# ScissorJack-ever/AlayaLite

Measured on AMD Instinct MI355X. Metric: QPS @ recall@10>=0.95, GIST-960 L2, 1M base / 1k queries, higher is better.
Workload: dtype f32

## Files before the change

alayalite_amd/csrc/capi.cpp:

```cpp
#include "../../include/alaya_hip.h"

#include <hip/hip_runtime_api.h>

#include <algorithm>
#include <cfloat>
#include <cmath>
#include <cstring>
#include <memory>
#include <mutex>
#include <stdexcept>
#include <limits>
#include <string>
#include <thread>
#include <vector>

#include "build_kernels.h"
#include "graph_update.h"
#include "hnsw_build.h"
#include "flat_bound.h"
#include "flat_kernels.h"
#include <cstdlib>
#include "screen_bound.h"
#include "search_kernels.h"

// ... 100 lines not shown
  uint32_t hash_log2_override = 0;
  int helpers_mode = -1;
  DevBuf help_stats;
  uint64_t help_stats_slots = 0;
  struct ScreenCopy {
    DevBuf rows, err;
    uint64_t cap = 0;
    bool ready = false;
    bool failed = false;
  };
  ScreenCopy screen_copy[2];
  uint32_t screen_format = 0;
  DevBuf screen_stats;
  uint64_t screen_stats_slots = 0;
  uint32_t last_grid = 0, last_waves = 0;
  int visited_mode_override = 0;
  int num_cus = 0;
  uint64_t capacity = 0;
  std::unique_ptr<alaya_amd::HostGraph> upd_graph;
  std::unique_ptr<alaya_amd::RowMirror> upd_rows;
  std::unique_ptr<alaya_amd::UpdateContext> upd_ctx;
  hipStream_t stream = nullptr;
  hipEvent_t scratch_ev = nullptr;
  hipStream_t scratch_stream = nullptr;
  bool scratch_used = false;
  uint64_t device_bytes() const {
    return base.bytes + valid.bytes + l0.bytes + levels.bytes + upper_off.bytes +
           upper_edges.bytes + eps.bytes + overflow.bytes + dirty.bytes + stab.bytes + codes.bytes + sq_min.bytes +
           sq_max.bytes;
  }
// ... 229 lines not shown
      const size_t probe = search_wave_lds_bytes(ix->stride, ef, 12, true);
      hip_check(search_occupancy(resolve_search_variant(r), p.ip, 1, probe, &b1), "occupancy");
      const uint64_t resident1 = static_cast<uint64_t>(std::max(1, b1)) * static_cast<uint64_t>(stream_cus(ix, stream));
      if (nq > resident1 && 2 * nq <= 3 * resident1) r.want |= kModeTwoWaves;
    }
  }
  if (ensure_screen(ix, p, p.sq8_order == 0 && plain, stream)) r.want |= kModeScreen;
  return r;
}

struct SearchPlan {
  const alaya_amd::SearchVariant *variant;
  int W;
  size_t lds;
  int grid;
};

SearchPlan plan_search(alaya_index *ix, SearchParams &p, alaya_amd::SearchRequest r, uint64_t nq, uint32_t ef,
                       hipStream_t stream) {
  using namespace alaya_amd;
  SearchPlan plan{};
  for (;;) {
    plan.variant = &resolve_search_variant(r);
    const int mode = plan.variant->mode;
    if ((r.want & kModeStamp) != 0 && (mode & kModeStamp) == 0)
      throw ArgError("no stamped search kernel for dim " + std::to_string(ix->dim) +
                     (p.sq8_order ? " SQ8 (order " + std::to_string(p.sq8_order) + ")" : std::string(" f32")) +
                     ": see the variant list in search_variants.h");
    p.help = (mode & kModeHelp) != 0;
    p.two_waves = (mode & kModeTwoWaves) != 0;
    p.screen = (mode & kModeScreen) != 0 ? ix->screen_format : 0u;
// ... 14 lines not shown
        fits = false;
      }
    }
    plan.lds = search_shared_lds_bytes(ix->stride, p.sq8_order != 0) + static_cast<size_t>(plan.W) * p.wave_lds +
               (p.help ? kHelpBoardBytes : 0);
    if (!p.help || (fits && plan.lds <= kLdsPerCu)) break;
    r.want &= ~kModeHelp;
  }
  if (plan.lds > kLdsPerCu) throw ArgError("ef / dim too large for the LDS budget");
  int per_cu = 0;
  hip_check(search_occupancy(*plan.variant, p.ip, plan.W, plan.lds, &per_cu), "occupancy");
  per_cu = static_cast<int>(std::max<uint64_t>(1, std::min<uint64_t>(per_cu, max_search_waves_per_cu() / plan.W)));
  const uint64_t cus = static_cast<uint64_t>(stream_cus(ix, stream));
  const uint64_t blocks_needed = p.help ? static_cast<uint64_t>(per_cu) * cus : (nq + plan.W - 1) / plan.W;
  plan.grid = static_cast<int>(std::max<uint64_t>(1, std::min<uint64_t>(blocks_needed, static_cast<uint64_t>(per_cu) * cus)));
  return plan;
}

void do_search(alaya_index *ix, const float *d_q, uint64_t nq, uint32_t k, uint32_t ef,
               uint32_t *d_ids, float *d_dists, uint32_t *d_cnt, hipStream_t stream,
               uint64_t *d_stamps = nullptr, bool sq8 = false, uint32_t fill_id = 0) {
  if (!ix->base.ptr) throw ArgError("index has no base vectors");
  if (!ix->has_graph) throw ArgError("index has no graph");
  if (ef == 0) throw ArgError("ef must be >= 1");
  if (k == 0 || nq == 0) return;
  if (ix->graph_n > ix->n) throw ArgError("graph has more nodes than base vectors");
  SearchParams p = base_params(ix);
  p.l0 = ix->l0.as<uint32_t>();
  p.R = ix->R;
  p.dedup_edges = ix->dedup;
// ... 23 lines not shown
    p.sq_max = ix->sq_max.as<float>();
  }
  p.stab_log2 = spill_table_log2(p.sq8_order, std::max<uint32_t>(1, ceil_log2(std::max<uint64_t>(ix->n, 2))), ef);
  if (const char *e = std::getenv("ALAYA_HELP_FLAGS")) p.help_flags = static_cast<uint32_t>(std::strtoul(e, nullptr, 10));
  const SearchPlan plan = plan_search(ix, p, search_request(ix, p, nq, ef, stream), nq, ef, stream);
  if (p.screen >= 2) {
    p.screen_u8 = ix->screen_copy[1].rows.as<uint8_t>();
  } else if (p.screen) {
    p.screen_rows = ix->screen_copy[0].rows.as<uint16_t>();
    p.screen_err = ix->screen_copy[0].err.as<float>();
  }
  scratch_acquire(ix, stream);
  const uint64_t searchers = static_cast<uint64_t>(plan.grid) * plan.W;
  prepare_spill(ix, p, searchers, stream);
  ix->last_grid = static_cast<uint32_t>(plan.grid);
  ix->last_waves = static_cast<uint32_t>(plan.W);
  ix->help_stats_slots = p.help ? searchers : 0;
  if (p.help) {
    ix->help_stats.reserve(searchers * 12);
    p.help_stats = ix->help_stats.as<uint32_t>();
  }
  ix->screen_stats_slots = p.screen ? searchers : 0;
  if (p.screen) {
    ix->screen_stats.reserve(searchers * 8);
    p.screen_stats = ix->screen_stats.as<uint32_t>();
  }
  ix->work.reserve(4);
  p.work_counter = ix->work.as<uint32_t>();
  hip_check(hipMemsetAsync(p.work_counter, 0, 4, stream), "hipMemsetAsync");
  hip_check(alaya_amd::launch_search(*plan.variant, p, plan.grid, plan.W, plan.lds, stream), "search launch");
  scratch_release(ix, stream);
}

uint32_t screen_default(uint32_t dim) {
  return (dim == 512 || dim == 768 || dim == 960 || dim == 1024) ? 3u : 0u;
}

void screen_fill(alaya_index *ix, uint32_t format, uint64_t first, uint64_t count, hipStream_t stream) {
  alaya_index::ScreenCopy &c = ix->screen_copy[format - 1];
  hip_check(format == 2 ? alaya_amd::launch_screen_rows_u8(ix->base.as<float>(), first, count, ix->stride,
                                                           c.rows.as<uint8_t>(), stream)
                        : alaya_amd::launch_screen_rows(ix->base.as<float>(), first, count, ix->stride,
                                                        c.rows.as<uint16_t>(), c.err.as<float>(), stream),
            "screening copy");
}
// ... 1449 lines not shown

int alaya_stream_destroy(void *stream) {
  return guarded([&] {
    if (stream) hip_check(hipStreamDestroy(static_cast<hipStream_t>(stream)), "hipStreamDestroy");
  });
}

int alaya_index_last_launch(const alaya_index *ix, uint32_t *workgroups, uint32_t *waves_per_group) {
  return guarded([&] {
    if (!ix) throw ArgError("null index");
    if (workgroups) *workgroups = ix->last_grid;
    if (waves_per_group) *waves_per_group = ix->last_waves;
  });
}

int alaya_index_set_helpers(alaya_index *ix, int mode) {
  return guarded([&] {
    if (!ix) throw ArgError("null index");
    if (mode < -1 || mode > 1) throw ArgError("helpers mode must be -1 (automatic), 0 (off) or 1 (on)");
    ix->helpers_mode = mode;
  });
}

int alaya_index_help_stats(alaya_index *ix, uint64_t *memo_dists, uint64_t *memo_expansions, uint64_t *helper_rows) {
  return guarded_scratch(ix, [&] {
    if (!ix) throw ArgError("null index");
    uint64_t m = 0, x = 0, r = 0;
    if (ix->help_stats_slots) {
      set_device(ix);
      scratch_drain(ix);
// ... 174 lines not shown
```

alayalite_amd/csrc/pybind_module.cpp:

```cpp
#include <pybind11/numpy.h>
#include <pybind11/pybind11.h>
#include <pybind11/stl.h>

#include <algorithm>
#include <cmath>
#include <cstring>
#include <fstream>
#include <memory>
#include <queue>
#include <stdexcept>
#include <string>
#include <vector>

#include "../../include/alaya_hip.h"

extern "C" int alaya_index_flat_diag(alaya_index *, const float *, uint64_t, uint32_t, int, uint32_t *, float *,
                                     uint32_t *, uint32_t *, void *);
#include "host_distance.h"

namespace py = pybind11;

namespace alaya_py {

enum class IndexType { FLAT = 0, HNSW = 1, NSG = 2, FUSION = 3, QG = 4 };
// ... 253 lines not shown
  void set_helpers(int m) { check(alaya_index_set_helpers(ix_, m)); }
  py::tuple last_launch() {
    uint32_t g = 0, w = 0;
    check(alaya_index_last_launch(ix_, &g, &w));
    return py::make_tuple(g, w);
  }
  py::tuple help_stats() {
    uint64_t m = 0, x = 0, r = 0;
    check(alaya_index_help_stats(ix_, &m, &x, &r));
    return py::make_tuple(m, x, r);
  }
  py::tuple screen_stats() {
    uint64_t a = 0, b = 0;
    check(alaya_index_screen_stats(ix_, &a, &b));
    return py::make_tuple(a, b);
  }
  void set_rerank_mode(int m) {
    if (m != 1 && m != 2) throw std::invalid_argument("rerank mode must be 1 (reference) or 2 (corrected)");
    rerank_mode_ = m;
  }
  int rerank_mode() const { return rerank_mode_; }
  py::array device_distances(py::array queries, py::array_t<uint32_t> ids) {
    py::array q = prepare_queries(queries);
    py::array_t<uint32_t, py::array::c_style | py::array::forcecast> idc(ids);
    const uint64_t nq = q.shape(0);
    const uint32_t n = static_cast<uint32_t>(idc.size());
    py::array_t<float> out({static_cast<py::ssize_t>(nq), static_cast<py::ssize_t>(n)});
    check(alaya_index_distances(ix_, static_cast<const float *>(q.data()), nq, idc.data(), n,
                                out.mutable_data()));
    return out;
// ... 544 lines not shown
  py::tuple last_launch() {
    uint32_t g = 0, w = 0;
    check(alaya_index_last_launch(ix_, &g, &w));
    return py::make_tuple(g, w);
  }
  py::tuple help_stats() {
    uint64_t m = 0, x = 0, r = 0;
    check(alaya_index_help_stats(ix_, &m, &x, &r));
    return py::make_tuple(m, x, r);
  }
  py::tuple screen_stats() {
    uint64_t a = 0, b = 0;
    check(alaya_index_screen_stats(ix_, &a, &b));
    return py::make_tuple(a, b);
  }
  py::tuple profile_search(py::array_t<float, py::array::c_style | py::array::forcecast> q, uint32_t k,
                           uint32_t ef, int space) {
    const uint64_t nq = q.shape(0);
    py::array_t<uint32_t> ids({static_cast<py::ssize_t>(nq), static_cast<py::ssize_t>(k)});
    py::array_t<uint32_t> c({static_cast<py::ssize_t>(nq), static_cast<py::ssize_t>(4)});
    py::array_t<uint64_t> st({static_cast<py::ssize_t>(nq), static_cast<py::ssize_t>(8)});
    check(alaya_index_profile_search(ix_, q.data(), nq, k, ef, space, ids.mutable_data(), c.mutable_data(),
                                     st.mutable_data()));
    return py::make_tuple(ids, c, st);
  }
  uint64_t device_bytes() const {
    uint64_t b = 0;
    check(alaya_index_info(ix_, nullptr, nullptr, nullptr, nullptr, &b));
    return b;
  }
// ... 65 lines not shown
      .def("batch_search_with_distance", &PyIndexInterface::batch_search_with_distance,
           py::arg("queries"), py::arg("topk"), py::arg("ef"), py::arg("num_threads"))
      .def("exact_search", &PyIndexInterface::exact_search, py::arg("queries"), py::arg("topk"))
      .def("save", &PyIndexInterface::save, py::arg("index_path"), py::arg("data_path"),
           py::arg("quant_path") = std::string())
      .def("load", &PyIndexInterface::load, py::arg("index_path"), py::arg("data_path"),
           py::arg("quant_path") = std::string())
      .def("get_data_dim", &PyIndexInterface::get_data_dim)
      .def("last_counters", &PyIndexInterface::last_counters)
      .def("set_hash_log2", &PyIndexInterface::set_hash_log2)
      .def("set_visited_mode", &PyIndexInterface::set_visited_mode)
      .def("set_helpers", &PyIndexInterface::set_helpers)
      .def("last_launch", &PyIndexInterface::last_launch)
      .def("help_stats", &PyIndexInterface::help_stats)
      .def("screen_stats", &PyIndexInterface::screen_stats)
      .def("set_rerank_mode", &PyIndexInterface::set_rerank_mode)
      .def("rerank_mode", &PyIndexInterface::rerank_mode)
      .def("device_distances", &PyIndexInterface::device_distances)
      .def("graph_arrays", &PyIndexInterface::graph_arrays);


  py::class_<Graph, std::shared_ptr<Graph>>(m, "Graph")
      .def_static("build", &Graph::build, py::arg("data"), py::arg("metric") = 0, py::arg("R") = 32u,
                  py::arg("ef_construction") = 100u, py::arg("num_threads") = 1u, py::arg("seed") = 100u)
      .def_static("load", &Graph::load, py::arg("path"), py::arg("id_bytes") = 4)
      .def_static("from_arrays", &Graph::from_arrays, py::arg("l0"), py::arg("levels"), py::arg("upper_off"),
                  py::arg("upper_edges"), py::arg("upper_R"), py::arg("ep"), py::arg("eps") = py::none())
      .def("save", &Graph::save, py::arg("path"), py::arg("id_bytes") = 4, py::arg("capacity") = 0u)
      .def("arrays", &Graph::arrays);
  py::class_<DeviceIndex, std::shared_ptr<DeviceIndex>>(m, "DeviceIndex")
      .def(py::init<int>(), py::arg("device") = 0)
      .def("set_base", &DeviceIndex::set_base, py::arg("rows"), py::arg("metric") = 0, py::arg("valid") = py::none())
      .def("set_graph", &DeviceIndex::set_graph)
      .def("build_graph", &DeviceIndex::build_graph, py::arg("R") = 32, py::arg("ef_construction") = 100,
           py::arg("seed") = 100, py::arg("batch_div") = 0, py::arg("max_batch") = 0, py::arg("refine") = 2)
      .def("search", &DeviceIndex::search, py::arg("queries"), py::arg("k"), py::arg("ef"))
      .def("search_device", &DeviceIndex::search_device)
      .def("shard_search_device", &DeviceIndex::shard_search_device)
      .def("distances", &DeviceIndex::distances)
      .def("set_hash_log2", &DeviceIndex::set_hash_log2)
      .def("set_visited_mode", &DeviceIndex::set_visited_mode)
      .def("set_helpers", &DeviceIndex::set_helpers)
      .def("last_launch", &DeviceIndex::last_launch)
      .def("help_stats", &DeviceIndex::help_stats)
      .def("screen_stats", &DeviceIndex::screen_stats)
      .def("flat_search", &DeviceIndex::flat_search, py::arg("queries"), py::arg("k"))
      .def("flat_search_device", &DeviceIndex::flat_search_device)
      .def("flat_diag", &DeviceIndex::flat_diag)
      .def("flat_contraction", &DeviceIndex::flat_contraction)
      .def("search_sq8_device", &DeviceIndex::search_sq8_device)
      .def("shard_search_sq8_device", &DeviceIndex::shard_search_sq8_device)
      .def("set_sq8", &DeviceIndex::set_sq8, py::arg("codes"), py::arg("min"), py::arg("max"), py::arg("order") = 2)
      .def("search_sq8", &DeviceIndex::search_sq8, py::arg("queries"), py::arg("k"), py::arg("ef"),
           py::arg("rerank") = 1, py::arg("rerank_queries") = py::none())
      .def("profile_search", &DeviceIndex::profile_search, py::arg("q"), py::arg("k"), py::arg("ef"),
           py::arg("space") = 0)
      .def("device_bytes", &DeviceIndex::device_bytes);
  m.def("sq8_train", [](py::array_t<float, py::array::c_style | py::array::forcecast> data) {
    const uint32_t d = static_cast<uint32_t>(data.shape(1));
    py::array_t<float> mn(d), mx(d);
// ... 103 lines not shown
```

alayalite_amd/csrc/search_device.h:

```cpp
#pragma once
#include <hip/hip_runtime.h>

#include <cfloat>
#include <cstdint>

#include "screen_bound.h"
#include "search_kernels.h"

namespace alaya_amd {
namespace {

constexpr uint32_t kEmpty = 0xffffffffu;
constexpr uint32_t kChecked = 0x80000000u;
constexpr uint32_t kIdMask = 0x7fffffffu;

__device__ __forceinline__ int lane_id() { return __lane_id(); }

__device__ __forceinline__ void wave_sync() {
  __builtin_amdgcn_fence(__ATOMIC_SEQ_CST, "wavefront");
  __builtin_amdgcn_wave_barrier();
}

__device__ __forceinline__ uint64_t ballot(bool p) { return __ballot(p); }

// ... 479 lines not shown
  Q.a2 = read_lane(a2, 0) + read_lane(a2, 32);
  Q.lo = lo;
  Q.scale = scale;
  Q.err = screen_u8_err(read_lane(sum, 0) + read_lane(sum, 32), p.stride, bad);
  return Q;
}

template <int kXor, int kN>
__device__ __forceinline__ void screen_fold(uint32_t *v, bool upper) {
#pragma unroll
  for (int i = 0; i < kN / 2; ++i) {
    const uint32_t keep = upper ? v[i + kN / 2] : v[i];
    const uint32_t send = upper ? v[i] : v[i + kN / 2];
    v[i] = keep + lane_xor<kXor>(send);
  }
}

template <int kChunks, typename Hook>
__device__ __forceinline__ void screen_dots_int(const SearchParams &p, const uint4 qc, const uint32_t *ids, int n,
                                                uint32_t *out, Hook after_issue) {
  constexpr int kPieces = 2 * kChunks;
  const int lane = lane_id();
  const uint32_t rec = screen_u8_record_bytes(p.stride);
  const uint32_t piece = kScreenU8Header + 16u * static_cast<uint32_t>(lane < kPieces ? lane : kPieces - 1);
  const int mine = ((lane & 1) << 4) | ((lane & 2) << 2) | (lane & 4) | ((lane & 8) >> 2) | ((lane & 16) >> 4);
  for (int base = 0; base < n; base += 32) {
    const uint32_t id = ids[base + lane < n ? base + lane : base];
    uint4 y[32];
#pragma unroll
    for (int r = 0; r < 32; ++r) {
// ... 807 lines not shown
```

alayalite_amd/csrc/search_kernels.h:

```cpp
#pragma once
#include <hip/hip_runtime_api.h>

#include <cstddef>
#include <cstdint>

#include "search_variants.h"

namespace alaya_amd {

struct SearchParams {
  const float *base;
  uint64_t n;
  uint32_t dim;
  uint32_t stride;
  const uint32_t *valid;
  bool ip;
  bool generic;
  const uint32_t *l0;
  uint32_t R;
  bool dedup_edges;
  const uint32_t *levels;
  const uint64_t *upper_off;
  const uint32_t *upper_edges;
  uint32_t upper_R;
// ... 27 lines not shown
  int sq8_order;
  const uint8_t *codes;
  uint32_t code_stride;
  const float *sq_min;
  const float *sq_max;
  uint32_t help;
  uint32_t help_flags;
  uint32_t memo_off;
  uint32_t two_waves;
  uint32_t *help_stats;
  uint32_t screen;
  const uint16_t *screen_rows;
  const float *screen_err;
  const uint8_t *screen_u8;
  uint32_t *screen_stats;
};

struct RerankParams {
  const uint32_t *search_ids;
  uint32_t k;
  uint32_t n_src;
  uint32_t n_take;
  uint32_t zeros;
  uint32_t fill_id;
  uint32_t *out_ids;
  float *out_dists;
};

constexpr uint32_t kVisWide = 0xffffffffu;
constexpr size_t kHelpBoardBytes = 256;
#ifndef ALAYA_HELP_DEPTH
// ... 29 lines not shown
```

alayalite_amd/csrc/search_kernels.hip:

```cpp
#include <hip/hip_runtime.h>

#include <cfloat>
#include <cstdint>

#include "screen_bound.h"
#include "search_kernels.h"
#include "search_device.h"

#ifndef ALAYA_MIN_WAVES_SQ8
#define ALAYA_MIN_WAVES_SQ8 -1
#endif
#ifndef ALAYA_MIN_WAVES_NARROW
#define ALAYA_MIN_WAVES_NARROW 0
#endif
#ifndef ALAYA_MIN_WAVES_WIDE
#define ALAYA_MIN_WAVES_WIDE 0
#endif
template <int kSpace>
constexpr bool space_sq8() { return kSpace == 1 || kSpace == 2; }
template <int kSpace>
constexpr bool space_tab() { return kSpace == 2; }

template <int kChunks, int kSpace, int kMode = 0>
constexpr int search_min_waves() {
// ... 425 lines not shown
      if (want) L.cid[slot] = v;
      wave_sync();
      space_distances<kIP, kChunks, kSpace>(p, Lt, L.cid, n, L.cd);
      if (lane == 0) b->own[wave].rows += static_cast<uint32_t>(n);
      if (want) {
        const uint64_t e = (static_cast<uint64_t>(seq) << 32) | __float_as_uint(L.cd[slot]);
        __hip_atomic_store(memo + (static_cast<uint32_t>(t) * kHelpSlots + s) * R + lane, e, __ATOMIC_RELAXED,
                           __HIP_MEMORY_SCOPE_WORKGROUP);
      }
      wave_sync();
    }
    if (!worked) __builtin_amdgcn_s_sleep(4);
  }
}

template <bool kIP, int kChunks, int kMode, int kSpace = 0>
__global__ void __launch_bounds__(256)
    __attribute__((amdgpu_waves_per_eu(search_min_waves<kChunks, kSpace, kMode>() ? search_min_waves<kChunks, kSpace, kMode>() : 1,
                                       8))) hnsw_search_kernel(SearchParams p) {
  extern __shared__ __attribute__((aligned(16))) unsigned char smem[];
  constexpr bool kStamp = (kMode & kModeStamp) != 0;
  constexpr bool kCheck = (kMode & kModeCheck) != 0;
  constexpr bool kHelp = (kMode & kModeHelp) != 0;
  constexpr int kRows = (kMode & kModeTwoWaves) != 0 ? 1 : 0;
  constexpr bool kScreen = (kMode & kModeScreen) != 0;
  static_assert(!kScreen || (kSpace == 0 && !kIP && !kHelp && kChunks >= 16 && kChunks % 2 == 0), "screen: wide f32 L2 rows");
  constexpr int kScreenRows = (kMode & kModeTwoWaves) != 0 ? 2 : 4;
  constexpr int kScreenRowsU8 = 4;
  uint32_t n_screened = 0, n_screened_out = 0;
  const int lane = lane_id();
  const int wave = static_cast<int>(threadIdx.x >> 6);
  const int W = static_cast<int>(blockDim.x >> 6);
  const Lds L = carve_lds<kSpace>(p, smem, wave);
  fill_shared<kSpace>(p, L);
  HelpBoard *board = kHelp ? help_board(p, smem, W) : nullptr;
  HelpMine mine;
  if constexpr (kHelp) {
    if constexpr (ALAYA_HELP_PRIO > 0) __builtin_amdgcn_s_setprio(ALAYA_HELP_PRIO);
    if (threadIdx.x == 0) help_board_init(board);
    __syncthreads();
    for (int s = 0; s < kHelpSlots; ++s) mine.node[s] = kEmpty, mine.seq[s] = 0u;
    mine.next_seq = 0u;
    mine.memo_wave = -1;
  }
  const uint64_t bit_words = (p.n + 31) / 32;
  const uint64_t slot = static_cast<uint64_t>(blockIdx.x) * (blockDim.x >> 6) + wave;
  uint32_t *slot_bits = p.overflow_bits + slot * bit_words;
  uint32_t *slot_dirty = p.dirty_words + slot * p.dirty_cap;
  uint16_t *slot_stab = (space_tab<kSpace>() && p.spill_table) ? p.spill_table + (slot << p.stab_log2) : nullptr;

  bool first_round = true;
  for (;;) {
    uint32_t qi = 0;
    if (kHelp && first_round) {
      qi = static_cast<uint32_t>(wave) * gridDim.x + blockIdx.x;
    } else {
      if (lane == 0) qi = atomicAdd(p.work_counter, 1u);
      qi = read_lane(qi, 0) + (kHelp ? static_cast<uint32_t>(W) * gridDim.x : 0u);
    }
    first_round = false;
    if (qi >= p.nq) break;
    if constexpr (kHelp) mine_reset(board, wave, mine);

    uint64_t st[8] = {0, 0, 0, 0, 0, 0, 0, 0};
    uint64_t t_prev = kStamp ? __builtin_readcyclecounter() : 0;
    const uint64_t t_begin = t_prev;
    auto stamp = [&](int slot) {
      if constexpr (kStamp) {
        const uint64_t now = __builtin_readcyclecounter();
        st[slot] += now - t_prev;
        t_prev = now;
      }
    };
    Visited vs;
    PoolState ps;
    uint32_t n_dist = 0, n_expand = 0, n_dist_up = 0, n_hops_up = 0;
    query_begin<kIP, kChunks, kSpace, kRows>(p, L, qi, slot_bits, slot_dirty, slot_stab, vs, ps, n_dist_up, n_hops_up);
    ScreenQuery sq{};
    if constexpr (kScreen) {
      if (p.screen == 3) sq = screen_query_codes<kChunks>(p, L.q);
    }

    stamp(0);
    uint32_t pred = kEmpty, pred_v = kEmpty;
    constexpr bool kSpillPrefetch = kSpace != 0;
    constexpr bool kRegMerge = kSpace == 0 && kChunks > 0 && kChunks <= 8;
    uint32_t pre_u = kEmpty;
    uint64_t pre_lo = 0ull, pre_hi = 0ull;
    while (ps.cur < ps.size) {
      uint32_t c1 = kEmpty, c2 = kEmpty;
      const uint32_t u = pool_pop<kHelp>(ps, L, &c1, &c2);
      ++n_expand;
      uint32_t look = 0u;
      if constexpr (kHelp) {
        if (mine.memo_wave < 0 && (n_expand & 3u) == 1u) {
          const uint32_t hw = help_word(board);
          if ((hw >> 8) != 0u) mine.memo_wave = static_cast<int>(hw >> 8) - 1;
        }
        if (mine.memo_wave >= 0) {
#pragma unroll
          for (int hs = 0; hs < kHelpSlots; ++hs)
            if (mine.node[hs] == u) look = (mine.seq[hs] << 2) | static_cast<uint32_t>(hs);
          mine_request(board, wave, mine, u, c1, c2);
        }
      }
#ifndef ALAYA_FINE_STAMPS
      if (kStamp && vs.spilled) st[5]++;
// ... 38 lines not shown
      }
      pre_u = kEmpty;
      pre_lo = pre_hi = 0ull;
      const uint64_t fm = ballot(fresh);
      const int nf = __popcll(fm);
      pred = ps.cur < ps.size ? (L.pi[ps.cur] & kIdMask) : kEmpty;
      if (pred != kEmpty && lane < static_cast<int>(p.R)) pred_v = p.l0[static_cast<uint64_t>(pred) * p.R + lane];
#ifdef ALAYA_FINE_STAMPS
      stamp(5);
#else
      stamp(2);
#endif
      if (nf == 0) continue;
      const uint32_t slot = __popcll(fm & ((1ull << lane) - 1ull));
      if (fresh) L.cid[slot] = v;
      const uint32_t *dist_ids = L.cid;
      bool compute = true;
      if constexpr (kHelp) {
        if (look != 0u) {
          const uint32_t seq = look >> 2;
          const int hs = static_cast<int>(look & 3u);
          const uint64_t *memo = help_memo<kSpace>(p, smem, mine.memo_wave) +
                                 (static_cast<uint32_t>(wave) * kHelpSlots + hs) * p.R;
          uint64_t e = 0ull;
          if (fresh) e = __hip_atomic_load(memo + lane, __ATOMIC_RELAXED, __HIP_MEMORY_SCOPE_WORKGROUP);
          const bool got = fresh && static_cast<uint32_t>(e >> 32) == seq;
          help_retire(board, wave, hs, seq);
          uint32_t *ids2 = reinterpret_cast<uint32_t *>(L.sd);
          if (fresh) {
            ids2[slot] = got ? kEmpty : v;
// ... 14 lines not shown
          if (vs.spilled && pred != kEmpty && !(p.spill_flags & 1u)) {
            if (p.spill_flags & 4u) __builtin_amdgcn_s_waitcnt(0);
            spill_prefetch(vs, pred_v, lane < static_cast<int>(p.R), pre_lo, pre_hi);
            pre_u = pred;
          }
        }
      };
      int nd = nf;
      if constexpr (kScreen) {
        if (ps.size == ps.ef) {
          const float tau = L.pd[ps.size - 1];
          const bool in = lane < nf;
          const uint32_t c = in ? L.cid[lane] : 0u;
          float e_row = 0.f;
          float lb3 = 0.f;
          if (p.screen == 3) {
            const uint8_t *rp = p.screen_u8 + static_cast<uint64_t>(c) * screen_u8_record_bytes(p.stride);
            const float4 head = *reinterpret_cast<const float4 *>(rp);
            const uint2 sums = *reinterpret_cast<const uint2 *>(rp + screen_u8_sums_offset(p.stride));
            screen_dots_int<kChunks>(p, sq.codes, L.cid, nf, reinterpret_cast<uint32_t *>(L.cd), second_level_prefetch);
            lb3 = screen_int_bound(p.stride, sq.err, sq.lo, sq.scale, sq.a1, sq.a2, head.x, head.y, head.z, sums.x, sums.y,
                                   __float_as_uint(L.cd[lane]));
          } else if (p.screen == 2) {
            if (in) e_row = *reinterpret_cast<const float *>(p.screen_u8 + static_cast<uint64_t>(c) * screen_u8_record_bytes(p.stride));
            screen_distances_u8<kChunks, kScreenRowsU8>(p, L.q, L.cid, nf, L.cd, second_level_prefetch);
          } else {
            if (in) e_row = p.screen_err[c];
            screen_distances<kChunks, kScreenRows>(p, L.q, L.cid, nf, L.cd, second_level_prefetch);
          }
          bool keep = false;
          if (in) {
// ... 30 lines not shown
      stamp(3);
      n_dist += nf;
      const bool has = lane < nd;
      const uint32_t cid = has ? L.cid[lane] : 0u;
      const float cd = has ? L.cd[lane] : 0.f;
      wave_sync();
      pool_merge<kRegMerge>(ps, L, has, cid, cd, [&](uint32_t nx) {
        if (nx != pred) {
          const uint32_t old_pred = pred;
          (void)old_pred;
          pred = nx;
          if (lane < static_cast<int>(p.R)) pred_v = p.l0[static_cast<uint64_t>(nx) * p.R + lane];
          if constexpr (kHelp) {
            if (mine.memo_wave >= 0) mine_request(board, wave, mine, kEmpty, nx, old_pred);
          }
        }
      }
#ifdef ALAYA_FINE_STAMPS
      , [&]() { stamp(7); }
#endif
      );
      stamp(4);
    }

    query_end(p, L, ps, qi, n_dist, n_expand, n_dist_up, n_hops_up);
    visit_end(vs);
    if constexpr (kStamp) {
      st[6] = __builtin_readcyclecounter() - t_begin;
      if (lane < 8) p.stamps[static_cast<uint64_t>(qi) * 8 + lane] = st[lane & 7];
    }
    wave_sync();
  }
  if constexpr (kHelp) {
    help_siblings<kIP, kChunks, kSpace>(p, smem, L, board, wave, W);
    if (p.help_stats != nullptr && lane == 0) {
      p.help_stats[3 * slot] = board->own[wave].hits;
      p.help_stats[3 * slot + 1] = board->own[wave].skips;
      p.help_stats[3 * slot + 2] = board->own[wave].rows;
    }
  }
  if constexpr (kScreen) {
    if (p.screen_stats != nullptr && lane == 0) {
      p.screen_stats[2 * slot] = n_screened;
      p.screen_stats[2 * slot + 1] = n_screened_out;
    }
  }
}

__global__ void __launch_bounds__(256) screen_rows_kernel(const float *base, uint64_t first, uint64_t count,
                                                          uint32_t stride, uint16_t *out_rows, float *out_err) {
  const int lane = lane_id();
  const uint64_t waves = static_cast<uint64_t>(gridDim.x) * (blockDim.x >> 6);
  for (uint64_t r = static_cast<uint64_t>(blockIdx.x) * (blockDim.x >> 6) + (threadIdx.x >> 6); r < count; r += waves) {
// ... 301 lines not shown
```

include/alaya_hip.h:

```cpp
#ifndef ALAYA_HIP_H_
#define ALAYA_HIP_H_

#include <stddef.h>
#include <stdint.h>

#ifdef __cplusplus
extern "C" {
#endif

#define ALAYA_OK 0
#define ALAYA_ERR_ARG 1
#define ALAYA_ERR_RUNTIME 2
#define ALAYA_ERR_DEVICE 3

#define ALAYA_METRIC_L2 0
#define ALAYA_METRIC_IP 1
#define ALAYA_METRIC_COS 2
#define ALAYA_DIST_GENERIC 0x100

typedef struct alaya_index alaya_index;
typedef struct alaya_graph alaya_graph;

const char *alaya_last_error(void);
const char *alaya_build_info(void);
// ... 76 lines not shown
                           uint64_t *helper_rows);
int alaya_index_screen_stats(alaya_index *ix, uint64_t *screened, uint64_t *screened_out);
int alaya_screen_lower_bound(const float *d_tilde, const float *e_row, uint64_t n, uint32_t dim, float *out);
int alaya_screen_u8_quantize(const float *rows, uint64_t n, uint32_t dim, uint8_t *codes, float *header,
                             float *values);
int alaya_screen_int_bound(const float *queries, const float *rows, uint64_t n, uint32_t dim, float *d_in,
                           float *e_sum, float *bound, uint32_t *sums);
int alaya_flat_ip_slack(int contraction, uint32_t k_acc, const float *q_norm2, const int *q_exp, uint64_t n,
                        float b_max, int base_exp, float *out);
int alaya_flat_ip_proven(const float *kth_d, const float *cutoff, const float *slack, uint64_t n, uint8_t *out);
int alaya_search_variant(uint32_t dim, int ip, int sq8_order, int generic, uint32_t wanted_mode, int *space,
                         uint32_t *chunks, uint32_t *mode, uint32_t *has_mode);
int alaya_search_variant_at(uint32_t index, int *space, uint32_t *chunks, uint32_t *mode, int *l2_only,
                            uint32_t *count);
int alaya_index_last_launch(const alaya_index *ix, uint32_t *workgroups, uint32_t *waves_per_group);
int alaya_index_info(const alaya_index *ix, uint64_t *n, uint32_t *dim, uint32_t *stride,
                     int *metric, uint64_t *device_bytes);

#ifdef __cplusplus
}
#endif
#endif
```

Before: 316,700.

## Add scout wave that precomputes screening bounds for upcoming graph expansions

Pairs each search wave with a low-priority scout wave in the same workgroup. Through an LDS board the search wave posts the nodes it is likely to expand next, and the scout computes their neighbours' u8 screening lower bounds ahead of time. When the search wave reaches that node it reuses the memoized bounds instead of doing the udot4 screening pass itself. This targets screening latency on the critical path, at the cost of doubling the waves per workgroup, extra LDS, polling and synchronisation overhead, and redundant work when its predictions miss.

```diff
diff --git a/alayalite_amd/csrc/capi.cpp b/alayalite_amd/csrc/capi.cpp
--- a/alayalite_amd/csrc/capi.cpp
+++ b/alayalite_amd/csrc/capi.cpp
@@ -138,6 +138,9 @@
   DevBuf screen_stats;
   uint64_t screen_stats_slots = 0;
   uint32_t last_grid = 0, last_waves = 0;
+  uint32_t last_lds = 0, last_hash_log2 = 0, last_compact = 0, last_per_cu = 0, last_scout = 0;
+  DevBuf scout_stats;
+  uint64_t scout_stats_slots = 0;
   int visited_mode_override = 0;
   int num_cus = 0;
   uint64_t capacity = 0;
@@ -397,7 +400,21 @@
   int W;
   size_t lds;
   int grid;
+  int per_cu;
 };
+
+uint32_t scout_default(uint32_t dim) { return (dim == 768 || dim == 960) ? alaya_amd::kScoutOn : 0u; }
+
+uint32_t scout_requested(uint32_t dim) {
+  const char *e = std::getenv("ALAYA_SEARCH_SCOUT");
+  const int asked = e && e[0] ? std::atoi(e) : -1;
+  uint32_t f = asked < 0 ? scout_default(dim) : (asked == 1 ? alaya_amd::kScoutOn : (asked == 2 ? alaya_amd::kScoutOn | alaya_amd::kScoutVerify : 0u));
+  if (f != 0u) {
+    const char *m = std::getenv("ALAYA_SEARCH_SCOUT_MISS");
+    if (m && std::atoi(m) != 0) f |= alaya_amd::kScoutMiss;
+  }
+  return f;
+}
 
 SearchPlan plan_search(alaya_index *ix, SearchParams &p, alaya_amd::SearchRequest r, uint64_t nq, uint32_t ef,
                        hipStream_t stream) {
@@ -442,6 +459,27 @@
   const uint64_t cus = static_cast<uint64_t>(stream_cus(ix, stream));
   const uint64_t blocks_needed = p.help ? static_cast<uint64_t>(per_cu) * cus : (nq + plan.W - 1) / plan.W;
   plan.grid = static_cast<int>(std::max<uint64_t>(1, std::min<uint64_t>(blocks_needed, static_cast<uint64_t>(per_cu) * cus)));
+  plan.per_cu = per_cu;
+  p.scout = 0u;
+  const uint32_t scout = scout_requested(ix->dim);
+  if (scout != 0u && p.screen == 3u && !p.ip && !p.two_waves && !p.help && plan.W == 1 && ix->R <= kScoutR &&
+      (plan.variant->mode & ~kModeScreen) == 0 && search_has_two_waves(ix->dim, p.sq8_order, ix->generic) &&
+      !helpers_requested(ix, p, nq, cus)) {
+    SearchRequest r2 = r;
+    r2.want |= kModeTwoWaves;
+    const SearchVariant &v2 = resolve_search_variant(r2);
+    const size_t lds2 = plan.lds + kScoutBoardBytes;
+    int per_cu2 = 0;
+    if (v2.mode == (kModeScreen | kModeTwoWaves) && lds2 <= kLdsPerCu)
+      hip_check(search_occupancy(v2, false, 2, lds2, &per_cu2), "occupancy");
+    if (per_cu2 >= per_cu && nq <= static_cast<uint64_t>(per_cu) * cus) {
+      plan.variant = &v2;
+      plan.lds = lds2;
+      p.scout = scout;
+      if (const char *e = std::getenv("ALAYA_SEARCH_SCOUT_GRID"))
+        plan.grid = std::max(1, std::min(plan.grid, std::atoi(e)));
+    }
+  }
   return plan;
 }
 
@@ -495,7 +533,18 @@
   const uint64_t searchers = static_cast<uint64_t>(plan.grid) * plan.W;
   prepare_spill(ix, p, searchers, stream);
   ix->last_grid = static_cast<uint32_t>(plan.grid);
-  ix->last_waves = static_cast<uint32_t>(plan.W);
+  const int wg_waves = p.scout ? 2 * plan.W : plan.W;
+  ix->last_waves = static_cast<uint32_t>(wg_waves);
+  ix->last_lds = static_cast<uint32_t>(plan.lds);
+  ix->last_hash_log2 = p.hash_log2;
+  ix->last_compact = p.vis_rbits != alaya_amd::kVisWide ? 1u : 0u;
+  ix->last_per_cu = static_cast<uint32_t>(plan.per_cu);
+  ix->last_scout = p.scout;
+  ix->scout_stats_slots = p.scout ? searchers : 0;
+  if (p.scout) {
+    ix->scout_stats.reserve(searchers * 16);
+    p.scout_stats = ix->scout_stats.as<uint32_t>();
+  }
   ix->help_stats_slots = p.help ? searchers : 0;
   if (p.help) {
     ix->help_stats.reserve(searchers * 12);
@@ -509,7 +558,7 @@
   ix->work.reserve(4);
   p.work_counter = ix->work.as<uint32_t>();
   hip_check(hipMemsetAsync(p.work_counter, 0, 4, stream), "hipMemsetAsync");
-  hip_check(alaya_amd::launch_search(*plan.variant, p, plan.grid, plan.W, plan.lds, stream), "search launch");
+  hip_check(alaya_amd::launch_search(*plan.variant, p, plan.grid, wg_waves, plan.lds, stream), "search launch");
   scratch_release(ix, stream);
 }
 
@@ -1989,6 +2038,37 @@
   });
 }
 
+int alaya_index_last_plan(const alaya_index *ix, uint32_t *lds_bytes, uint32_t *hash_log2, uint32_t *compact,
+                          uint32_t *groups_per_cu, uint32_t *scout) {
+  return guarded([&] {
+    if (!ix) throw ArgError("null index");
+    if (lds_bytes) *lds_bytes = ix->last_lds;
+    if (hash_log2) *hash_log2 = ix->last_hash_log2;
+    if (compact) *compact = ix->last_compact;
+    if (groups_per_cu) *groups_per_cu = ix->last_per_cu;
+    if (scout) *scout = ix->last_scout;
+  });
+}
+
+int alaya_index_scout_stats(alaya_index *ix, uint64_t *expansions, uint64_t *hits, uint64_t *records,
+                            uint64_t *mismatches) {
+  return guarded_scratch(ix, [&] {
+    if (!ix) throw ArgError("null index");
+    uint64_t t[4] = {0, 0, 0, 0};
+    if (ix->scout_stats_slots) {
+      set_device(ix);
+      scratch_drain(ix);
+      std::vector<uint32_t> h(4 * ix->scout_stats_slots);
+      hip_check(hipMemcpy(h.data(), ix->scout_stats.ptr, h.size() * 4, hipMemcpyDeviceToHost), "D2H");
+      for (uint64_t i = 0; i < h.size(); ++i) t[i & 3] += h[i];
+    }
+    if (expansions) *expansions = t[0];
+    if (hits) *hits = t[1];
+    if (records) *records = t[2];
+    if (mismatches) *mismatches = t[3];
+  });
+}
+
 int alaya_index_set_helpers(alaya_index *ix, int mode) {
   return guarded([&] {
     if (!ix) throw ArgError("null index");
diff --git a/alayalite_amd/csrc/pybind_module.cpp b/alayalite_amd/csrc/pybind_module.cpp
--- a/alayalite_amd/csrc/pybind_module.cpp
+++ b/alayalite_amd/csrc/pybind_module.cpp
@@ -291,6 +291,25 @@
     uint64_t a = 0, b = 0;
     check(alaya_index_screen_stats(ix_, &a, &b));
     return py::make_tuple(a, b);
+  }
+  py::tuple scout_stats() {
+    uint64_t e = 0, h = 0, r = 0, m = 0;
+    check(alaya_index_scout_stats(ix_, &e, &h, &r, &m));
+    return py::make_tuple(e, h, r, m);
+  }
+  py::dict last_plan() {
+    uint32_t g = 0, w = 0, lds = 0, hl = 0, c = 0, pc = 0, sc = 0;
+    check(alaya_index_last_launch(ix_, &g, &w));
+    check(alaya_index_last_plan(ix_, &lds, &hl, &c, &pc, &sc));
+    py::dict d;
+    d["workgroups"] = g;
+    d["waves_per_group"] = w;
+    d["lds_bytes"] = lds;
+    d["hash_log2"] = hl;
+    d["compact"] = c != 0;
+    d["groups_per_cu"] = pc;
+    d["scout"] = sc;
+    return d;
   }
   void set_rerank_mode(int m) {
     if (m != 1 && m != 2) throw std::invalid_argument("rerank mode must be 1 (reference) or 2 (corrected)");
@@ -865,6 +884,25 @@
     check(alaya_index_screen_stats(ix_, &a, &b));
     return py::make_tuple(a, b);
   }
+  py::tuple scout_stats() {
+    uint64_t e = 0, h = 0, r = 0, m = 0;
+    check(alaya_index_scout_stats(ix_, &e, &h, &r, &m));
+    return py::make_tuple(e, h, r, m);
+  }
+  py::dict last_plan() {
+    uint32_t g = 0, w = 0, lds = 0, hl = 0, c = 0, pc = 0, sc = 0;
+    check(alaya_index_last_launch(ix_, &g, &w));
+    check(alaya_index_last_plan(ix_, &lds, &hl, &c, &pc, &sc));
+    py::dict d;
+    d["workgroups"] = g;
+    d["waves_per_group"] = w;
+    d["lds_bytes"] = lds;
+    d["hash_log2"] = hl;
+    d["compact"] = c != 0;
+    d["groups_per_cu"] = pc;
+    d["scout"] = sc;
+    return d;
+  }
   py::tuple profile_search(py::array_t<float, py::array::c_style | py::array::forcecast> q, uint32_t k,
                            uint32_t ef, int space) {
     const uint64_t nq = q.shape(0);
@@ -960,6 +998,8 @@
       .def("last_launch", &PyIndexInterface::last_launch)
       .def("help_stats", &PyIndexInterface::help_stats)
       .def("screen_stats", &PyIndexInterface::screen_stats)
+      .def("scout_stats", &PyIndexInterface::scout_stats)
+      .def("last_plan", &PyIndexInterface::last_plan)
       .def("set_rerank_mode", &PyIndexInterface::set_rerank_mode)
       .def("rerank_mode", &PyIndexInterface::rerank_mode)
       .def("device_distances", &PyIndexInterface::device_distances)
@@ -990,6 +1030,8 @@
       .def("last_launch", &DeviceIndex::last_launch)
       .def("help_stats", &DeviceIndex::help_stats)
       .def("screen_stats", &DeviceIndex::screen_stats)
+      .def("scout_stats", &DeviceIndex::scout_stats)
+      .def("last_plan", &DeviceIndex::last_plan)
       .def("flat_search", &DeviceIndex::flat_search, py::arg("queries"), py::arg("k"))
       .def("flat_search_device", &DeviceIndex::flat_search_device)
       .def("flat_diag", &DeviceIndex::flat_diag)
diff --git a/alayalite_amd/csrc/search_device.h b/alayalite_amd/csrc/search_device.h
--- a/alayalite_amd/csrc/search_device.h
+++ b/alayalite_amd/csrc/search_device.h
@@ -517,6 +517,41 @@
     const uint32_t send = upper ? v[i] : v[i + kN / 2];
     v[i] = keep + lane_xor<kXor>(send);
   }
+}
+
+__device__ __forceinline__ int screen_pass_row(int lane) {
+  return ((lane & 1) << 4) | ((lane & 2) << 2) | (lane & 4) | ((lane & 8) >> 2) | ((lane & 16) >> 4);
+}
+
+template <int kChunks, typename Hook>
+__device__ __forceinline__ uint32_t screen_dots_pass(const SearchParams &p, const uint4 qc, uint32_t id, Hook after_issue) {
+  constexpr int kPieces = 2 * kChunks;
+  const int lane = lane_id();
+  const uint32_t rec = screen_u8_record_bytes(p.stride);
+  const uint32_t piece = kScreenU8Header + 16u * static_cast<uint32_t>(lane < kPieces ? lane : kPieces - 1);
+  uint4 y[32];
+#pragma unroll
+  for (int r = 0; r < 32; ++r) {
+    const uint8_t *rp = p.screen_u8 + static_cast<uint64_t>(read_lane(id, r)) * rec;
+    y[r] = *reinterpret_cast<const uint4 *>(rp + piece);
+  }
+  __builtin_amdgcn_sched_barrier(0);
+  after_issue();
+  uint32_t acc[32];
+#pragma unroll
+  for (int r = 0; r < 32; ++r) {
+    uint32_t a = __builtin_amdgcn_udot4(qc.x, y[r].x, 0u, false);
+    a = __builtin_amdgcn_udot4(qc.y, y[r].y, a, false);
+    a = __builtin_amdgcn_udot4(qc.z, y[r].z, a, false);
+    acc[r] = __builtin_amdgcn_udot4(qc.w, y[r].w, a, false);
+    if ((r & 7) == 7) __builtin_amdgcn_sched_barrier(0);
+  }
+  screen_fold<1, 32>(acc, (lane & 1) != 0);
+  screen_fold<2, 16>(acc, (lane & 2) != 0);
+  screen_fold<4, 8>(acc, (lane & 4) != 0);
+  screen_fold<8, 4>(acc, (lane & 8) != 0);
+  screen_fold<16, 2>(acc, (lane & 16) != 0);
+  return acc[0] + static_cast<uint32_t>(__builtin_amdgcn_ds_bpermute((lane ^ 32) << 2, static_cast<int>(acc[0])));
 }
 
 template <int kChunks, typename Hook>
diff --git a/alayalite_amd/csrc/search_kernels.h b/alayalite_amd/csrc/search_kernels.h
--- a/alayalite_amd/csrc/search_kernels.h
+++ b/alayalite_amd/csrc/search_kernels.h
@@ -65,7 +65,13 @@
   const float *screen_err;
   const uint8_t *screen_u8;
   uint32_t *screen_stats;
+  uint32_t scout;
+  uint32_t *scout_stats;
 };
+constexpr uint32_t kScoutOn = 1, kScoutVerify = 2, kScoutMiss = 4;
+constexpr uint32_t kScoutSlots = 3;
+constexpr uint32_t kScoutR = 32;
+constexpr size_t kScoutBoardBytes = kScoutSlots * (kScoutR * 4 + 8 + 4) + 20;
 
 struct RerankParams {
   const uint32_t *search_ids;
diff --git a/alayalite_amd/csrc/search_kernels.hip b/alayalite_amd/csrc/search_kernels.hip
--- a/alayalite_amd/csrc/search_kernels.hip
+++ b/alayalite_amd/csrc/search_kernels.hip
@@ -463,6 +463,121 @@
   }
 }
 
+constexpr uint32_t kScoutDone = 0xffffffffu;
+constexpr uint32_t kScoutMissing = 0xffffffffu;
+constexpr uint64_t kScoutNoMatch = 1ull << 63;
+struct ScoutBoard {
+  uint64_t tag[kScoutSlots];
+  uint32_t bound[kScoutSlots][kScoutR];
+  uint32_t req[kScoutSlots];
+  uint32_t state;
+  uint32_t stat[3];
+  uint32_t pad;
+};
+static_assert(sizeof(ScoutBoard) == kScoutBoardBytes && kScoutSlots == 3, "board size");
+
+__device__ __forceinline__ ScoutBoard *scout_board(const SearchParams &p, unsigned char *smem, int n_search, int i) {
+  return reinterpret_cast<ScoutBoard *>(smem + search_shared_lds_bytes(p.stride, p.sq8_order != 0) +
+                                        static_cast<size_t>(n_search) * p.wave_lds) + i;
+}
+
+template <typename T>
+__device__ __forceinline__ T lds_load(const T *a) {
+  return __hip_atomic_load(a, __ATOMIC_RELAXED, __HIP_MEMORY_SCOPE_WORKGROUP);
+}
+template <typename T, typename U>
+__device__ __forceinline__ void lds_store(T *a, U v) {
+  __hip_atomic_store(a, static_cast<T>(v), __ATOMIC_RELAXED, __HIP_MEMORY_SCOPE_WORKGROUP);
+}
+__device__ __forceinline__ void lds_order() { asm volatile("" ::: "memory"); }
+
+__device__ __forceinline__ uint64_t scout_key(uint32_t epoch, uint32_t node) {
+  return (static_cast<uint64_t>(epoch & 0x7fffffffu) << 32) | node;
+}
+
+__device__ __forceinline__ void scout_post(ScoutBoard *b, int first, int n, uint32_t x0, uint32_t x1, uint32_t x2) {
+  const int lane = lane_id();
+  if (lane < n) lds_store(&b->req[first + lane], lane == 0 ? x0 : (lane == 1 ? x1 : x2));
+}
+
+template <int kChunks>
+__device__ void scout_loop(const SearchParams &p, const Lds &Ls, ScoutBoard *b, uint32_t *stats) {
+  const int lane = lane_id();
+  const int mine = screen_pass_row(lane);
+  const int R = static_cast<int>(p.R);
+  const uint32_t rec = screen_u8_record_bytes(p.stride);
+  const bool miss = (p.scout & kScoutMiss) != 0u;
+  __builtin_amdgcn_s_setprio(0);
+  ScreenQuery sq{};
+  uint32_t sq_epoch = 0u;
+  uint32_t records = 0u;
+  for (;;) {
+    const uint32_t e = read_lane(lds_load(&b->state), 0);
+    if (e == kScoutDone) break;
+    if (e == 0u) {
+      __builtin_amdgcn_s_sleep(8);
+      continue;
+    }
+    if (e != sq_epoch) {
+      lds_order();
+      sq = screen_query_codes<kChunks>(p, Ls.q);
+      lds_order();
+      sq_epoch = read_lane(lds_load(&b->state), 0) == e ? e : 0u;
+      continue;
+    }
+    uint32_t rq = kEmpty;
+    uint64_t tg = 0ull;
+    if (lane < static_cast<int>(kScoutSlots)) {
+      rq = lds_load(&b->req[lane]);
+      tg = lds_load(&b->tag[lane]);
+    }
+    lds_order();
+    if (read_lane(lds_load(&b->state), 0) != sq_epoch) continue;
+    const uint32_t u = read_lane(rq, 0), c1 = read_lane(rq, 1), c2 = read_lane(rq, 2);
+    const uint64_t ku = scout_key(e, u), k1 = scout_key(e, c1), k2 = scout_key(e, c2);
+    tg &= ~kScoutNoMatch;
+    const bool have1 = ballot(tg == k1) != 0ull, have2 = ballot(tg == k2) != 0ull;
+    uint32_t node = kEmpty;
+    if (!miss && c1 != kEmpty && !have1) {
+      node = c1;
+    } else if (c2 != kEmpty && !have2) {
+      node = c2;
+    }
+    const uint64_t spare = ballot(lane < static_cast<int>(kScoutSlots) && tg != ku && tg != k1 && tg != k2);
+    if (node == kEmpty || spare == 0ull) {
+      __builtin_amdgcn_s_sleep(8);
+      continue;
+    }
+    const int row = __ffsll(static_cast<unsigned long long>(spare)) - 1;
+    const uint32_t v = lane < R ? p.l0[static_cast<uint64_t>(node) * p.R + lane] : kEmpty;
+    const uint64_t endm = ballot(lane < R && v == kEmpty);
+    const int cnt = endm ? __ffsll(static_cast<unsigned long long>(endm)) - 1 : R;
+    bool want = lane < cnt;
+    want = want && !sibling_visited<0>(p, Ls, 0, v, want);
+    const uint64_t wm = ballot(want);
+    if (lane == 0) lds_store(&b->tag[row], 0ull);
+    lds_order();
+    uint32_t lb_bits = kScoutMissing;
+    if (wm != 0ull) {
+      const uint32_t v0 = read_lane(v, __ffsll(static_cast<unsigned long long>(wm)) - 1);
+      const uint32_t id = want ? v : v0;
+      const uint32_t idm = static_cast<uint32_t>(__builtin_amdgcn_ds_bpermute(mine << 2, static_cast<int>(id)));
+      const uint8_t *rp = p.screen_u8 + static_cast<uint64_t>(idm) * rec;
+      const float4 head = *reinterpret_cast<const float4 *>(rp);
+      const uint2 sums = *reinterpret_cast<const uint2 *>(rp + screen_u8_sums_offset(p.stride));
+      const uint32_t ac = screen_dots_pass<kChunks>(p, sq.codes, id, NoHook());
+      const float lb = screen_int_bound(p.stride, sq.err, sq.lo, sq.scale, sq.a1, sq.a2, head.x, head.y, head.z, sums.x,
+                                        sums.y, ac);
+      if ((wm >> mine) & 1ull) lb_bits = __float_as_uint(lb);
+      records += static_cast<uint32_t>(__popcll(wm));
+    }
+    if (lane < 32 && mine < R) lds_store(&b->bound[row][mine], lb_bits);
+    lds_order();
+    if (lane == 0) lds_store(&b->tag[row], scout_key(e, node) | (miss ? kScoutNoMatch : 0ull));
+  }
+  if (stats != nullptr && lane == 0) stats[2] = records;
+}
+
 template <bool kIP, int kChunks, int kMode, int kSpace = 0>
 __global__ void __launch_bounds__(256)
     __attribute__((amdgpu_waves_per_eu(search_min_waves<kChunks, kSpace, kMode>() ? search_min_waves<kChunks, kSpace, kMode>() : 1,
@@ -479,7 +594,29 @@
   uint32_t n_screened = 0, n_screened_out = 0;
   const int lane = lane_id();
   const int wave = static_cast<int>(threadIdx.x >> 6);
-  const int W = static_cast<int>(blockDim.x >> 6);
+  constexpr bool kScout = kScreen && (kMode & kModeTwoWaves) != 0;
+  const bool scouting = kScout && p.scout != 0u;
+  const int W = static_cast<int>(blockDim.x >> 6) >> (scouting ? 1 : 0);
+  ScoutBoard *sboard = nullptr;
+  if constexpr (kScout) {
+    if (scouting) {
+      sboard = scout_board(p, smem, W, wave < W ? wave : wave - W);
+      if (wave < W && lane < static_cast<int>(kScoutSlots)) {
+        sboard->req[lane] = kEmpty;
+        sboard->tag[lane] = 0ull;
+        sboard->stat[lane] = 0u;
+        sboard->state = 0u;
+      }
+      __syncthreads();
+      if (wave >= W) {
+        const uint64_t sslot = static_cast<uint64_t>(blockIdx.x) * W + (wave - W);
+        scout_loop<kChunks>(p, carve_lds<kSpace>(p, smem, wave - W), sboard,
+                            p.scout_stats != nullptr ? p.scout_stats + 4 * sslot : nullptr);
+        return;
+      }
+      __builtin_amdgcn_s_setprio(2);
+    }
+  }
   const Lds L = carve_lds<kSpace>(p, smem, wave);
   fill_shared<kSpace>(p, L);
   HelpBoard *board = kHelp ? help_board(p, smem, W) : nullptr;
@@ -493,7 +630,7 @@
     mine.memo_wave = -1;
   }
   const uint64_t bit_words = (p.n + 31) / 32;
-  const uint64_t slot = static_cast<uint64_t>(blockIdx.x) * (blockDim.x >> 6) + wave;
+  const uint64_t slot = static_cast<uint64_t>(blockIdx.x) * W + wave;
   uint32_t *slot_bits = p.overflow_bits + slot * bit_words;
   uint32_t *slot_dirty = p.dirty_words + slot * p.dirty_cap;
   uint16_t *slot_stab = (space_tab<kSpace>() && p.spill_table) ? p.spill_table + (slot << p.stab_log2) : nullptr;
@@ -510,6 +647,13 @@
     first_round = false;
     if (qi >= p.nq) break;
     if constexpr (kHelp) mine_reset(board, wave, mine);
+    if constexpr (kScout) {
+      if (scouting) {
+        if (lane == 0) lds_store(&sboard->state, 0u);
+        lds_order();
+        scout_post(sboard, 0, 3, kEmpty, kEmpty, kEmpty);
+      }
+    }
 
     uint64_t st[8] = {0, 0, 0, 0, 0, 0, 0, 0};
     uint64_t t_prev = kStamp ? __builtin_readcyclecounter() : 0;
@@ -529,6 +673,12 @@
     if constexpr (kScreen) {
       if (p.screen == 3) sq = screen_query_codes<kChunks>(p, L.q);
     }
+    if constexpr (kScout) {
+      if (scouting) {
+        lds_order();
+        if (lane == 0) lds_store(&sboard->state, qi + 1u);
+      }
+    }
 
     stamp(0);
     uint32_t pred = kEmpty, pred_v = kEmpty;
@@ -538,8 +688,11 @@
     uint64_t pre_lo = 0ull, pre_hi = 0ull;
     while (ps.cur < ps.size) {
       uint32_t c1 = kEmpty, c2 = kEmpty;
-      const uint32_t u = pool_pop<kHelp>(ps, L, &c1, &c2);
+      const uint32_t u = pool_pop<kHelp || kScout>(ps, L, &c1, &c2);
       ++n_expand;
+      if constexpr (kScout) {
+        if (scouting && ps.size == ps.ef) scout_post(sboard, 0, 3, u, c1, c2);
+      }
       uint32_t look = 0u;
       if constexpr (kHelp) {
         if (mine.memo_wave < 0 && (n_expand & 3u) == 1u) {
@@ -608,6 +761,25 @@
       if (nf == 0) continue;
       const uint32_t slot = __popcll(fm & ((1ull << lane) - 1ull));
       if (fresh) L.cid[slot] = v;
+      bool memo_ok = false;
+      if constexpr (kScout) {
+        if (scouting && ps.size == ps.ef && p.screen == 3) {
+          const uint64_t key = scout_key(qi + 1u, u);
+          uint64_t tg = 0ull;
+          if (lane < static_cast<int>(kScoutSlots)) tg = lds_load(&sboard->tag[lane]);
+          const uint64_t rows = ballot(tg == key);
+          if (rows != 0ull) {
+            const int row = __ffsll(static_cast<unsigned long long>(rows)) - 1;
+            lds_order();
+            const uint32_t mb = lds_load(&sboard->bound[row][lane & static_cast<int>(kScoutR - 1)]);
+            lds_order();
+            const uint64_t again = lds_load(&sboard->tag[row]);
+            memo_ok = ballot(again != key || (fresh && (mb == kScoutMissing || lane >= static_cast<int>(kScoutR)))) == 0ull;
+            if (memo_ok && fresh) L.cd[slot] = __uint_as_float(mb);
+          }
+          if (lane == 0) lds_store(&sboard->req[0], kEmpty);
+        }
+      }
       const uint32_t *dist_ids = L.cid;
       bool compute = true;
       if constexpr (kHelp) {
@@ -652,7 +824,24 @@
           const uint32_t c = in ? L.cid[lane] : 0u;
           float e_row = 0.f;
           float lb3 = 0.f;
-          if (p.screen == 3) {
+          if (p.screen == 3 && kScout && memo_ok) {
+            lb3 = L.cd[lane];
+            if (lane == 0) sboard->stat[0] += 1u, sboard->stat[1] += 1u;
+            if (p.scout & kScoutVerify) {
+              const uint8_t *rp = p.screen_u8 + static_cast<uint64_t>(c) * screen_u8_record_bytes(p.stride);
+              const float4 head = *reinterpret_cast<const float4 *>(rp);
+              const uint2 sums = *reinterpret_cast<const uint2 *>(rp + screen_u8_sums_offset(p.stride));
+              wave_sync();
+              screen_dots_int<kChunks>(p, sq.codes, L.cid, nf, reinterpret_cast<uint32_t *>(L.cd), NoHook());
+              const float own = screen_int_bound(p.stride, sq.err, sq.lo, sq.scale, sq.a1, sq.a2, head.x, head.y, head.z,
+                                                 sums.x, sums.y, __float_as_uint(L.cd[lane]));
+              const uint32_t bad = static_cast<uint32_t>(__popcll(ballot(in && __float_as_uint(own) != __float_as_uint(lb3))));
+              if (lane == 0 && bad != 0u) sboard->stat[2] += bad;
+            }
+          } else if (p.screen == 3) {
+            if constexpr (kScout) {
+              if (scouting && lane == 0) sboard->stat[0] += 1u;
+            }
             const uint8_t *rp = p.screen_u8 + static_cast<uint64_t>(c) * screen_u8_record_bytes(p.stride);
             const float4 head = *reinterpret_cast<const float4 *>(rp);
             const uint2 sums = *reinterpret_cast<const uint2 *>(rp + screen_u8_sums_offset(p.stride));
@@ -713,6 +902,9 @@
           if constexpr (kHelp) {
             if (mine.memo_wave >= 0) mine_request(board, wave, mine, kEmpty, nx, old_pred);
           }
+          if constexpr (kScout) {
+            if (scouting && ps.size == ps.ef) scout_post(sboard, 1, 2, nx, old_pred, kEmpty);
+          }
         }
       }
 #ifdef ALAYA_FINE_STAMPS
@@ -736,6 +928,16 @@
       p.help_stats[3 * slot] = board->own[wave].hits;
       p.help_stats[3 * slot + 1] = board->own[wave].skips;
       p.help_stats[3 * slot + 2] = board->own[wave].rows;
+    }
+  }
+  if constexpr (kScout) {
+    if (scouting) {
+      if (lane == 0) lds_store(&sboard->state, kScoutDone);
+      if (p.scout_stats != nullptr && lane == 0) {
+        p.scout_stats[4 * slot] = sboard->stat[0];
+        p.scout_stats[4 * slot + 1] = sboard->stat[1];
+        p.scout_stats[4 * slot + 3] = sboard->stat[2];
+      }
     }
   }
   if constexpr (kScreen) {
diff --git a/include/alaya_hip.h b/include/alaya_hip.h
--- a/include/alaya_hip.h
+++ b/include/alaya_hip.h
@@ -114,6 +114,10 @@
 int alaya_search_variant_at(uint32_t index, int *space, uint32_t *chunks, uint32_t *mode, int *l2_only,
                             uint32_t *count);
 int alaya_index_last_launch(const alaya_index *ix, uint32_t *workgroups, uint32_t *waves_per_group);
+int alaya_index_last_plan(const alaya_index *ix, uint32_t *lds_bytes, uint32_t *hash_log2, uint32_t *compact,
+                          uint32_t *groups_per_cu, uint32_t *scout);
+int alaya_index_scout_stats(alaya_index *ix, uint64_t *expansions, uint64_t *hits, uint64_t *records,
+                            uint64_t *mismatches);
 int alaya_index_info(const alaya_index *ix, uint64_t *n, uint32_t *dim, uint32_t *stride,
                      int *metric, uint64_t *device_bytes);
 
```

Result: faster. 341,600 (median of 6 runs) (+7.8%).
